# Chemical118/TREW

Measured on NVIDIA B200. Metric: Gbases/s for trew short 5 32 at 1/2/4/8 B200; % of HBM roofline, higher is better.
Workload: dtype u64

## Files before the change

trew_b200/csrc/exact_thread.cuh:

```cuda
#pragma once
#include <stdint.h>

#if defined(__CUDACC__)
#define ET_HD __host__ __device__ __forceinline__
#define ET_FN __host__ __device__ __noinline__
#else
#define ET_HD inline
#define ET_FN inline
#endif

namespace trew {
namespace et {

typedef uint32_t u32;
typedef uint64_t u64;
typedef unsigned __int128 u128;

constexpr int kReadWords = 5;
constexpr int kMaxRead = 32 * kReadWords;
constexpr int kClsCap = 6;
constexpr int kClsSpill = kMaxRead - kClsCap;
constexpr int kApproxMaxWindows = 48;

enum {
    W_H = 0, W_L = W_H + kReadWords + 2, W_V = W_L + kReadWords + 2,
    W_PH = W_V + kReadWords, W_PL = W_PH + kReadWords + 2,
    W_WV = W_PL + kReadWords + 2, W_LINK = W_WV + kReadWords,
    W_CKEY = W_LINK + kReadWords
};
template <class K>
struct Lay {
    static constexpr int KW = (int)(sizeof(K) / 4);
    static constexpr int CT = W_CKEY + KW * kClsCap, WORDS = CT + kClsCap;
};
constexpr int kWorkWords = Lay<u64>::WORDS;

struct Mem {
    u32* base; int stride;
    ET_HD u32& operator[](int i) const { return base[i * stride]; }
};

ET_HD int popc(u32 x) {
#if defined(__CUDA_ARCH__)
    return __popc(x);
#else
    return __builtin_popcount(x);
#endif
}
ET_HD int ffs1(u32 x) {
#if defined(__CUDA_ARCH__)
    return __ffs(x) - 1;
#else
    return __builtin_ctz(x);
#endif
}
ET_HD u32 fshr(u32 lo, u32 hi, int sh) {
#if defined(__CUDA_ARCH__)
    return __funnelshift_r(lo, hi, sh);
#else
    sh &= 31;
    return sh ? (lo >> sh) | (hi << (32 - sh)) : lo;
#endif
}
ET_HD u32 brev32(u32 x) {
#if defined(__CUDA_ARCH__)
    return __brev(x);
#else
    x = ((x >> 1) & 0x55555555u) | ((x & 0x55555555u) << 1);
    x = ((x >> 2) & 0x33333333u) | ((x & 0x33333333u) << 2);
    x = ((x >> 4) & 0x0f0f0f0fu) | ((x & 0x0f0f0f0fu) << 4);
    x = ((x >> 8) & 0x00ff00ffu) | ((x & 0x00ff00ffu) << 8);
    return (x >> 16) | (x << 16);
#endif
}
ET_HD u32 lowmask(int bits) { return bits >= 32 ? 0xffffffffu : (bits <= 0 ? 0u : ((1u << bits) - 1u)); }
ET_HD u32 pxor32(u32 x) { x ^= x << 1; x ^= x << 2; x ^= x << 4; x ^= x << 8; x ^= x << 16; return x; }
ET_HD u64 spread(u32 x) {
    u64 v = x;
    v = (v | (v << 16)) & 0x0000FFFF0000FFFFULL;
    v = (v | (v << 8)) & 0x00FF00FF00FF00FFULL;
    v = (v | (v << 4)) & 0x0F0F0F0F0F0F0F0FULL;
    v = (v | (v << 2)) & 0x3333333333333333ULL;
    v = (v | (v << 1)) & 0x5555555555555555ULL;
    return v;
}

ET_FN u64 canon64(u64 w, int k) {
    const int sh = 2 * (k - 1);
    if (k <= 16) {
        u32 b = (u32)w, c = (u32)w;
        for (int r = 1; r < k; r++) { c = ((c & 3u) << sh) | (c >> 2); b = c < b ? c : b; }
        return b;
    }
    u64 best = w, cur = w;
    for (int r = 1; r < k; r++) { cur = ((cur & 3ULL) << sh) | (cur >> 2); best = cur < best ? cur : best; }
    return best;
}
ET_FN u128 canon128(u128 w, int k) {
    const int sh = 2 * (k - 1);
    u128 best = w, cur = w;
    for (int r = 1; r < k; r++) { cur = ((cur & 3) << sh) | (cur >> 2); best = cur < best ? cur : best; }
    return best;
}
ET_HD u64 canon(u64 w, int k) { return canon64(w, k); }
ET_HD u128 canon(u128 w, int k) { return k <= 32 ? (u128)canon64((u64)w, k) : canon128(w, k); }
ET_HD u64 crc(u64 w, int k) {
    const u32 lo = brev32((u32)w), hi = brev32((u32)(w >> 32));
    u64 x = ((u64)lo << 32) | hi;
    x = ((x >> 1) & 0x5555555555555555ULL) | ((x & 0x5555555555555555ULL) << 1);
    return canon64(~x >> (64 - 2 * k), k);
}
ET_HD u128 crc(u128 w, int k) {
    if (k <= 32) return (u128)crc((u64)w, k);
    u128 r = 0;
    for (int i = 0; i < k; i++) { r = (r << 2) | (3 - (w & 3)); w >>= 2; }
    return canon128(r, k);
}
ET_HD bool homo(u64 w, int k) {
    return k <= 1 || ((w ^ (w >> 2)) & ((1ULL << (2 * (k - 1))) - 1ULL)) == 0;
}
ET_HD bool homo(u128 w, int k) {
    return k <= 1 || ((w ^ (w >> 2)) & ((((u128)1) << (2 * (k - 1))) - 1)) == 0;
}

template <class K>
struct ClsSpill {
    K key[kClsSpill];
    unsigned short tot[kClsSpill], last[kClsSpill];
};

template <class K>
ET_HD K cls_key(Mem m, int q) {
    K v = 0;
    for (int i = Lay<K>::KW - 1; i >= 0; i--) v = (v << 16 << 16) | (K)m[W_CKEY + Lay<K>::KW * q + i];
    return v;
}
template <class K>
ET_HD void cls_put(Mem m, int q, K key) {
    for (int i = 0; i < Lay<K>::KW; i++) { m[W_CKEY + Lay<K>::KW * q + i] = (u32)key; key = key >> 16 >> 16; }
}

ET_HD u32 shr_plane(Mem m, int base, int j, int k) {
    if (k < 32) return fshr(m[base + j], m[base + j + 1], k);
    if (k == 32) return m[base + j + 1];
    if (k < 64) return fshr(m[base + j + 1], m[base + j + 2], k - 32);
    return m[base + j + 2];
}

ET_HD u64 raw_kmer(Mem m, int j, int b, int k, u64& hk, u64& lk, u64) {
    const u32 km = lowmask(k);
    const u32 h = fshr(m[W_H + j], m[W_H + j + 1], b) & km, l = fshr(m[W_L + j], m[W_L + j + 1], b) & km;
    hk = h; lk = l;
    return (spread(brev32(h) >> (32 - k)) << 1) | spread(brev32(l) >> (32 - k));
}
ET_HD u128 raw_kmer(Mem m, int j, int b, int k, u64& hk, u64& lk, u128) {
    if (k <= 32) return (u128)raw_kmer(m, j, b, k, hk, lk, (u64)0);
    const u64 km = k >= 64 ? ~0ULL : ((1ULL << k) - 1ULL);
    hk = ((u64)fshr(m[W_H + j], m[W_H + j + 1], b) | ((u64)fshr(m[W_H + j + 1], m[W_H + j + 2], b) << 32)) & km;
    lk = ((u64)fshr(m[W_L + j], m[W_L + j + 1], b) | ((u64)fshr(m[W_L + j + 1], m[W_L + j + 2], b) << 32)) & km;
    const u64 hr = (((u64)brev32((u32)hk) << 32) | brev32((u32)(hk >> 32))) >> (64 - k);
    const u64 lr = (((u64)brev32((u32)lk) << 32) | brev32((u32)(lk >> 32))) >> (64 - k);
    const u64 lo = (spread((u32)hr) << 1) | spread((u32)lr), hi = (spread((u32)(hr >> 32)) << 1) | spread((u32)(lr >> 32));
    return ((u128)hi << 64) | lo;
}

ET_HD u32 run_starts(Mem m, int j) {
    return m[W_WV + j] & ~((m[W_LINK + j] << 1) | (j ? m[W_LINK + j - 1] >> 31 : 0u));
}
ET_FN int prepare_runs(Mem m, int nw, int k) {
    for (int j = 0; j < nw; j++) {
        const u32 hs = shr_plane(m, W_H, j, k), ls = shr_plane(m, W_L, j, k);
        const u32 eq = ~((hs ^ m[W_H + j]) | (ls ^ m[W_L + j]));
        const u32 wvj = m[W_WV + j];
        const u32 nxt = (wvj >> 1) | (j + 1 < nw ? m[W_WV + j + 1] << 31 : 0u);
        m[W_LINK + j] = eq & wvj & nxt;
    }
    int runs = 0;
    for (int j = 0; j < nw; j++) runs += popc(run_starts(m, j));
    return runs;
}

template <class K>
ET_FN int classify_runs(Mem m, int runs, int k, ClsSpill<K>& x, bool approx, int T = 0, int need_min = 0) {
    int n = 0, ord = 0, j = 0, best = 0;
    const int slack = T - need_min;
    u32 wvj = m[W_WV], rr = run_starts(m, 0);
    for (int r = 0; r < runs; r++) {
        while (!rr) { ord += popc(wvj); j++; rr = run_starts(m, j); wvj = m[W_WV + j]; }
        {
            const int b = ffs1(rr);
            rr &= rr - 1;
            const u32 c0 = (u32)(ord + popc(wvj & ((1u << b) - 1u)));
            int jj = j;
            u32 z = ~m[W_LINK + j] & (0xffffffffu << b);
            while (!z) { jj++; z = ~m[W_LINK + jj]; }
            const u32 cnt = (u32)(32 * (jj - j) + ffs1(z) - b + 1);
            u64 hk, lk;
            K key = raw_kmer(m, j, b, k, hk, lk, (K)0);
            if (approx) key = (K)((u32)(popc((u32)hk) + popc((u32)(hk >> 32))) | ((u32)(popc((u32)lk) + popc((u32)(lk >> 32))) << 8) |
                                  ((u32)(popc((u32)(hk & lk)) + popc((u32)((hk & lk) >> 32))) << 16));
            else key = canon(key, k);
            const u32 last = c0 + cnt - 1u;
            int q = 0;
            const int nq = n < kClsCap ? n : kClsCap;
            while (q < nq && cls_key<K>(m, q) != key) q++;
            u32 tot = cnt;
            if (q < nq) {
                const u32 ct = (m[Lay<K>::CT + q] & 0xffff0000u) + (cnt << 16);
                m[Lay<K>::CT + q] = ct | last;
                tot = ct >> 16;
            } else if (n < kClsCap) {
                cls_put<K>(m, n, key); m[Lay<K>::CT + n] = (cnt << 16) | last;
                n++;
            } else {
                int s = 0;
                while (s < n - kClsCap && x.key[s] != key) s++;
                if (s < n - kClsCap) { tot = x.tot[s] + cnt; x.tot[s] = (unsigned short)tot; x.last[s] = (unsigned short)last; }
                else { x.key[s] = key; x.tot[s] = (unsigned short)cnt; x.last[s] = (unsigned short)last; n++; }
            }
            if (need_min > 0) {
                best = (int)tot > best ? (int)tot : best;
                if ((int)last + 1 - best > slack) return -1;
            }
        }
    }
    return n;
}

template <class K>
ET_FN int cls_max(Mem m, int n, const ClsSpill<K>& x, K& S) {
    u32 best = 0;
    S = 0;
    for (int q = 0; q < n && q < kClsCap; q++) {
        const u32 ct = m[Lay<K>::CT + q];
        const u32 score = ((ct >> 16) << 10) | (1023u - (ct & 0xffffu));
        if (score > best) { best = score; S = cls_key<K>(m, q); }
    }
    for (int q = 0; q < n - kClsCap; q++) {
        const u32 score = ((u32)x.tot[q] << 10) | (1023u - x.last[q]);
        if (score > best) { best = score; S = x.key[q]; }
    }
    return (int)(best >> 10);
}

ET_HD bool need_pass(const unsigned short* thr, u32 need, int M, int T) {
    const u32 mm = need & 0xffffu, t = need >> 16;
    return M >= (int)thr[T] && (t == 0u || (u32)M * t >= mm * (u32)T);
}

ET_HD int min_accept(const unsigned short* thr, u32 need, int T) {
    const u32 mm = need & 0xffffu, t = need >> 16;
    const int a = (int)thr[T], b = t ? (int)((mm * (u32)T + t - 1u) / t) : 0;
    return a > b ? a : b;
}

ET_HD void shrink_valid(Mem m, int nw) {
    for (int j = 0; j < nw; j++) m[W_WV + j] &= (m[W_WV + j] >> 1) | (j + 1 < nw ? m[W_WV + j + 1] << 31 : 0u);
}

template <class K>
ET_FN u32 scan_window(Mem m, int len, int kmin, int kmax, const unsigned short* thr_low, const unsigned short* thr_high, ClsSpill<K>& x,
                      K& S_h, K& S_l) {
    S_h = S_l = 0;
    if (kmax > len) kmax = len;
    if (kmax < kmin) return 0u;
    const int nw = (len + 31) >> 5;
    {
        u32 ch = 0, cl = 0, tph = 0, tpl = 0;
        for (int j = 0; j <= nw; j++) {
            const u32 ih = pxor32(m[W_H + j]) ^ ch, il = pxor32(m[W_L + j]) ^ cl;
            m[W_PH + j] = (ih << 1) | tph; m[W_PL + j] = (il << 1) | tpl;
            tph = ih >> 31; tpl = il >> 31;
            ch = 0u - tph; cl = 0u - tpl;
        }
        m[W_PH + nw + 1] = 0u; m[W_PL + nw + 1] = 0u;
    }
    for (int j = 0; j < nw; j++) m[W_WV + j] = m[W_V + j];
    for (int t = 1; t < kmin; t++) shrink_valid(m, nw);
    K blockedL = 0, blockedH = 0;
    u32 needL = 0, needH = 0;
    u32 res = 0;
    for (int k = kmin; k <= kmax; k++, shrink_valid(m, nw)) {
        const bool blkL = (bool)((blockedL >> k) & 1), blkH = (bool)((blockedH >> k) & 1);
        int T = 0, cH = 0, cL = 0, c11 = 0;
        for (int j = 0; j < nw; j++) {
            const u32 wvj = m[W_WV + j];
            const u32 dh = (shr_plane(m, W_PH, j, k) ^ m[W_PH + j]) & wvj;
            const u32 dl = (shr_plane(m, W_PL, j, k) ^ m[W_PL + j]) & wvj;
            T += popc(wvj); cH += popc(dh); cL += popc(dl); c11 += popc(dh & dl);
        }
        if (T == 0) break;
        if (blkL && blkH) continue;
        const int c10 = cH - c11, c01 = cL - c11, c00 = T - cH - cL + c11;
        int U = c00 > c01 ? c00 : c01;
        U = U > c10 ? U : c10;
        U = U > c11 ? U : c11;
        if (!((!blkL && need_pass(thr_low, needL, U, T)) || (!blkH && need_pass(thr_high, needH, U, T)))) continue;
        K S;
        const int runs = prepare_runs(m, nw, k);
        int need_min = 1 << 20;
        if (!blkL) need_min = min_accept(thr_low, needL, T);
        if (!blkH) { const int a = min_accept(thr_high, needH, T); need_min = a < need_min ? a : need_min; }
        if (runs > 3 && T <= kApproxMaxWindows) {
            const int na = classify_runs(m, runs, k, x, true, T, need_min);
            if (na < 0) continue;
            const int Mu = cls_max(m, na, x, S);
            if (!((!blkL && need_pass(thr_low, needL, Mu, T)) || (!blkH && need_pass(thr_high, needH, Mu, T)))) continue;
        }
        const int n = classify_runs(m, runs, k, x, false, T, need_min);
        if (n < 0) continue;
        const int M = cls_max(m, n, x, S);
        if (homo(S, k)) continue;
        const bool accL = !blkL && need_pass(thr_low, needL, M, T), accH = !blkH && need_pass(thr_high, needH, M, T);
        if (accL || accH) {
            K mm = 0;
            for (int j = k; j <= kmax; j += k) mm |= ((K)1) << j;
            const u32 need = (u32)M | ((u32)T << 16);
            if (accL) { res = (res & 0xffu) | ((u32)k << 8); needL = need; blockedL |= mm; S_l = S; }
            if (accH) { res = (res & 0xff00u) | (u32)k; needH = need; blockedH |= mm; S_h = S; }
        }
    }
    return res;
}

enum { T_F = 0, T_B = 2, T_O = 4 };

template <class K, class Emit>
ET_HD void emit_window_classes(Mem m, int len, int k, int table, bool folded, ClsSpill<K>& x, Emit& emit);

template <class K, class Load, class Emit>
ET_HD bool route_short_thread(Mem m, int n, u32 pm, int min_mer, int max_mer, const unsigned short* thr_low,
                              const unsigned short* thr_high, Load& load, Emit& emit) {
    if (n < 2 * min_mer) return true;
    if (max_mer > (int)(4 * sizeof(K)) || n > kMaxRead) return false;
    const int kmax = n / 4 < max_mer ? n / 4 : max_mer;
    const int llen = n / 2, rlen = (n + 1) / 2, roff = n - rlen;
    ClsSpill<K> x;
    u32 L = 0, R = 0;
    K sh, sl;
    const bool halves = n >= 4 * min_mer;
    for (u32 todo = halves ? pm & 3u : 0u; todo != 0u; todo &= todo - 1u) {
        const bool right = (todo & 1u) == 0u;
        const int len = right ? rlen : llen;
        load(0, right ? roff : 0, len);
        const u32 r = scan_window(m, len, min_mer, kmax, thr_low, thr_high, x, sh, sl);
        if (right) R = r; else L = r;
    }
    if (4 * max_mer > n) {
        const bool hc0 = ((L | R) & 0xffu) == 0u, hc1 = ((L | R) >> 8) == 0u;
        const u32 wbit = halves ? 4u : 1u;
        if ((hc0 || hc1) && (pm & wbit)) {
            const int lo = n / 4 + 1 > min_mer ? n / 4 + 1 : min_mer, hi = n / 2 < max_mer ? n / 2 : max_mer;
            load(0, 0, n);
            const u32 W = scan_window(m, n, lo, hi, thr_low, thr_high, x, sh, sl);
            for (int c = 0; c < 2; c++) {
                const int k = (int)((W >> (8 * c)) & 0xffu);
                if ((c == 0 ? hc0 : hc1) && k) emit_window_classes(m, n, k, T_O + c, false, x, emit);
            }
        }
    }
    if ((L | R) == 0u) return true;
    int cur_win = -1, cur_k = 0, ncls = 0, T = 0;
    for (int c = 0; c < 2; c++) {
        const int Lc = (int)((L >> (8 * c)) & 0xffu), Rc = (int)((R >> (8 * c)) & 0xffu);
        int win, k, table;
        if (Lc > 0 && Lc == Rc) { win = 2; k = Lc; table = T_O + c; }
        else if (Lc > 0) { win = 0; k = Lc; table = T_F + c; }
        else if (Rc > 0) { win = 1; k = Rc; table = T_B + c; }
        else continue;
        if (win != cur_win || k != cur_k) {
            const int off = win == 1 ? roff : 0, len = win == 2 ? n : (win == 0 ? llen : rlen), nw = (len + 31) >> 5;
            load(0, off, len);
            for (int j = 0; j < nw; j++) m[W_WV + j] = m[W_V + j];
            for (int t = 1; t < k; t++) shrink_valid(m, nw);
            T = 0;
            for (int j = 0; j < nw; j++) T += popc(m[W_WV + j]);
            ncls = 0;
            if (T) ncls = classify_runs(m, prepare_runs(m, nw, k), k, x, false);
            cur_win = win; cur_k = k;
        }
        if (T == 0) continue;
        const bool target = win == 2;
        if (target) {
            K S;
            const int M = cls_max(m, ncls, x, S);
            if (homo(S, k) || M < (int)(c == 0 ? thr_high : thr_low)[T]) continue;
        }
        for (int q = 0; q < ncls; q++) {
            K key = q < kClsCap ? cls_key<K>(m, q) : x.key[q - kClsCap];
            const u64 cnt = q < kClsCap ? (u64)(m[Lay<K>::CT + q] >> 16) : (u64)x.tot[q - kClsCap];
            if (target) { const K t = crc(key, k); key = t < key ? t : key; }
            emit(table, k, key, cnt);
        }
    }
    return true;
}

template <class K, class Emit>
ET_HD void emit_window_classes(Mem m, int len, int k, int table, bool folded, ClsSpill<K>& x, Emit& emit) {
    const int nw = (len + 31) >> 5;
    for (int j = 0; j < nw; j++) m[W_WV + j] = m[W_V + j];
    for (int t = 1; t < k; t++) shrink_valid(m, nw);
    int T = 0;
    for (int j = 0; j < nw; j++) T += popc(m[W_WV + j]);
    if (T == 0) return;
    const int ncls = classify_runs(m, prepare_runs(m, nw, k), k, x, false);
    for (int q = 0; q < ncls; q++) {
        K key = q < kClsCap ? cls_key<K>(m, q) : x.key[q - kClsCap];
        const u64 cnt = q < kClsCap ? (u64)(m[Lay<K>::CT + q] >> 16) : (u64)x.tot[q - kClsCap];
        if (folded) { const K t = crc(key, k); key = t < key ? t : key; }
        emit(table, k, key, cnt);
    }
}

template <class K, class Load, class Emit>
ET_HD bool route_pair_thread(Mem m, int n1, int n2, int min_mer, int max_mer, const unsigned short* thr_low,
                             const unsigned short* thr_high, Load& load, Emit& emit) {
    const int n = n1 < n2 ? n1 : n2;
    if (n < 2 * min_mer) return true;
    if (max_mer > (int)(4 * sizeof(K)) || n1 > kMaxRead || n2 > kMaxRead || 4 * max_mer > n) return false;
    const int kmax = n / 4 < max_mer ? n / 4 : max_mer;
    const int soff[5] = {0, 0, n1 - (n1 + 1) / 2, n2 - (n2 + 1) / 2, 0};
    const int slen[5] = {0, n1 / 2, (n1 + 1) / 2, (n2 + 1) / 2, n2 / 2};
    ClsSpill<K> x;
    u32 res[5] = {0, 0, 0, 0, 0};
    K S[5][2];
    bool have[5] = {false, false, false, false, false};
    auto window = [&](int t) { load(t <= 2 ? 0 : 1, soff[t], slen[t]); };
    auto scan = [&](int t) {
        if (have[t]) return;
        window(t);
        res[t] = scan_window(m, slen[t], min_mer, kmax, thr_low, thr_high, x, S[t][0], S[t][1]);
        have[t] = true;
    };
    int pseg[2][8], ptmp[2][8], np[2] = {0, 0};
    int si[2] = {1, 1}, km[2] = {0, 0};
    bool ended[2] = {false, false};
    K ks[2] = {0, 0};
    for (int ti = 1; ti <= 4 && !(ended[0] && ended[1]); ti++) {
        scan(ti);
        for (int c = 0; c < 2; c++) {
            const int k = (int)((res[ti] >> (8 * c)) & 0xffu);
            if (!ended[c] && k) { pseg[c][np[c]] = ti; ptmp[c][np[c]] = ti <= 2 ? 0 : 1; np[c]++; }
            bool ok = !ended[c] && k > 0;
            if (ok && ti != 1) {
                const K ds = ti > 2 ? crc(S[ti][c], k) : S[ti][c];
                ok = km[c] == k && ks[c] == ds;
            }
            if (ok) { si[c]++; km[c] = k; if (ti == 1) ks[c] = S[ti][c]; }
            else ended[c] = true;
        }
    }
    for (int c = 0; c < 2; c++) {
        if (si[c] == 5) {
            for (int e = 0; e < np[c]; e++) {
                const int sg = pseg[c][e];
                window(sg);
                emit_window_classes(m, slen[sg], (int)((res[sg] >> (8 * c)) & 0xffu), T_O + c, true, x, emit);
            }
        }
    }
    if (si[0] <= 4 || si[1] <= 4) {
        int sj[2] = {4, 4};
        km[0] = km[1] = 0; ended[0] = ended[1] = false;
        for (int tj = 4; tj >= 1 && !(ended[0] && ended[1]); tj--) {
            scan(tj);
            for (int c = 0; c < 2; c++) {
                const int k = (int)((res[tj] >> (8 * c)) & 0xffu);
                if (!ended[c] && k) { pseg[c][np[c]] = tj; ptmp[c][np[c]] = tj <= 2 ? 1 : 0; np[c]++; }
                bool ok = sj[c] >= si[c] && !ended[c] && k > 0;
                if (ok && tj != 4) {
                    const K ds = tj <= 2 ? crc(S[tj][c], k) : S[tj][c];
                    ok = km[c] == k && ks[c] == ds;
                }
                if (ok) { sj[c]--; km[c] = k; if (tj == 4) ks[c] = S[tj][c]; }
                else ended[c] = true;
            }
        }
    }
    for (int c = 0; c < 2; c++) {
        if (si[c] <= 4) {
            for (int e = 0; e < np[c]; e++) {
                const int sg = pseg[c][e];
                window(sg);
                emit_window_classes(m, slen[sg], (int)((res[sg] >> (8 * c)) & 0xffu), (ptmp[c][e] == 0 ? T_F : T_B) + c, false, x, emit);
            }
        }
    }
    return true;
}


struct LongGeom {
    int n, SL, snum, mid, bonus;
    ET_HD LongGeom(int n_, int SL_) : n(n_), SL(SL_), snum(n_ / SL_), mid((n_ / SL_ + 1) / 2), bonus(n_ % SL_) {}
    ET_HD int start(int t) const { return (t - 1) * SL + (t > mid ? bonus : 0); }
    ET_HD int len(int t) const { return SL + (t == mid ? bonus : 0); }
};

template <class Load>
ET_HD u32 long_slice_stats(Mem m, const LongGeom& g, int t, int min_mer, int max_mer, const unsigned short* thr_low,
                           const unsigned short* thr_high, Load& load, ClsSpill<u64>& x) {
    const int len = g.len(t);
    load(0, g.start(t), len);
    u64 sh, sl;
    return scan_window(m, len, min_mer, max_mer, thr_low, thr_high, x, sh, sl);
}

struct LongTask { unsigned short slice; unsigned char k, table_folded; };

template <class Stat, class Task>
ET_HD bool long_walk(const LongGeom& g, Stat& stat, Task& task) {
    const int snum = g.snum;
    const bool mid_ok = g.len(g.mid) <= kMaxRead;
    for (int pass = mid_ok ? 1 : 0; pass < 2; pass++) {
        int si[2] = {1, 1}, km[2] = {0, 0};
        bool ended[2] = {false, false};
        int nf = 0;
        for (int ti = 1; ti <= snum && !(ended[0] && ended[1]); ti++) {
            if (pass == 0 && ti == g.mid) return false;
            const u32 r = stat(ti);
            for (int c = 0; c < 2; c++) {
                const int k = (int)((r >> (8 * c)) & 0xffu);
                if (!ended[c] && k > 0 && (ti == 1 || km[c] == k)) { si[c]++; km[c] = k; }
                else ended[c] = true;
            }
            nf = ti;
        }
        if (pass == 1) {
            bool en[2] = {false, false};
            int kk[2] = {0, 0};
            const bool full[2] = {si[0] == snum + 1, si[1] == snum + 1};
            for (int ti = 1; ti <= nf; ti++) {
                const u32 r = stat(ti);
                for (int c = 0; c < 2; c++) {
                    const int k = (int)((r >> (8 * c)) & 0xffu);
                    if (!en[c] && k) task(LongTask{(unsigned short)ti, (unsigned char)k, (unsigned char)(((full[c] ? T_O : T_F) + c) | (full[c] ? 8 : 0))});
                    if (!en[c] && k > 0 && (ti == 1 || kk[c] == k)) kk[c] = k;
                    else en[c] = true;
                }
            }
        }
        if (si[0] <= snum || si[1] <= snum) {
            int sj[2] = {snum, snum};
            km[0] = km[1] = 0; ended[0] = ended[1] = false;
            for (int tj = snum; tj >= 1 && !(ended[0] && ended[1]); tj--) {
                if (pass == 0 && tj == g.mid) return false;
                const u32 r = stat(tj);
                for (int c = 0; c < 2; c++) {
                    const int k = (int)((r >> (8 * c)) & 0xffu);
                    if (pass == 1 && !ended[c] && k) task(LongTask{(unsigned short)tj, (unsigned char)k, (unsigned char)(T_B + c)});
                    if (sj[c] >= si[c] && !ended[c] && k > 0 && (tj == snum || km[c] == k)) { sj[c]--; km[c] = k; }
                    else ended[c] = true;
                }
            }
        }
    }
    return true;
}

template <class Load, class Emit>
ET_HD void long_emit(Mem m, const LongGeom& g, const LongTask& tk, Load& load, ClsSpill<u64>& x, Emit& emit) {
    const int len = g.len(tk.slice);
    load(0, g.start(tk.slice), len);
    emit_window_classes(m, len, tk.k, tk.table_folded & 7, (tk.table_folded & 8) != 0, x, emit);
}

}
}
```

Baseline: 986.2.

## Keep period planes in registers and memoize raw-kmer class lookups

The prefix-xor planes and the valid-window mask move out of strided scratch memory into fixed-size register arrays. A templated scan with compile-time word count (3 words for short windows) and unrolled signature counting replaces the strided loads. classify_runs adds a small memo of raw k-mers that maps repeats straight to their class slot, skipping canonicalisation and the linear key search. The blocked-period masks shrink to a narrower bit set. Together these cut local/global memory traffic and ALU work, at the cost of more register pressure and code size from the template instantiations.

```diff
diff --git a/trew_b200/csrc/exact_thread.cuh b/trew_b200/csrc/exact_thread.cuh
--- a/trew_b200/csrc/exact_thread.cuh
+++ b/trew_b200/csrc/exact_thread.cuh
@@ -8,6 +8,13 @@
 #define ET_HD inline
 #define ET_FN inline
 #endif
+#if defined(__CUDA_ARCH__)
+#define ET_UNROLL _Pragma("unroll")
+#define ET_NO_UNROLL _Pragma("unroll 1")
+#else
+#define ET_UNROLL
+#define ET_NO_UNROLL
+#endif
 
 namespace trew {
 namespace et {
@@ -24,8 +31,7 @@
 
 enum {
     W_H = 0, W_L = W_H + kReadWords + 2, W_V = W_L + kReadWords + 2,
-    W_PH = W_V + kReadWords, W_PL = W_PH + kReadWords + 2,
-    W_WV = W_PL + kReadWords + 2, W_LINK = W_WV + kReadWords,
+    W_WV = W_V + kReadWords, W_LINK = W_WV + kReadWords,
     W_CKEY = W_LINK + kReadWords
 };
 template <class K>
@@ -180,10 +186,20 @@
     return runs;
 }
 
+constexpr int kMemo = 4;
+#if defined(ET_MEMO_STATS) && !defined(__CUDA_ARCH__)
+inline long memo_runs = 0, memo_hits = 0;
+#define ET_MEMO_COUNT(hit) (memo_runs++, memo_hits += (hit) >= 0)
+#else
+#define ET_MEMO_COUNT(hit) ((void)0)
+#endif
 template <class K>
 ET_FN int classify_runs(Mem m, int runs, int k, ClsSpill<K>& x, bool approx, int T = 0, int need_min = 0) {
     int n = 0, ord = 0, j = 0, best = 0;
     const int slack = T - need_min;
+    K mraw[kMemo];
+    u32 mcls = 0;
+    int nm = 0;
     u32 wvj = m[W_WV], rr = run_starts(m, 0);
     for (int r = 0; r < runs; r++) {
         while (!rr) { ord += popc(wvj); j++; rr = run_starts(m, j); wvj = m[W_WV + j]; }
@@ -196,27 +212,50 @@
             while (!z) { jj++; z = ~m[W_LINK + jj]; }
             const u32 cnt = (u32)(32 * (jj - j) + ffs1(z) - b + 1);
             u64 hk, lk;
-            K key = raw_kmer(m, j, b, k, hk, lk, (K)0);
-            if (approx) key = (K)((u32)(popc((u32)hk) + popc((u32)(hk >> 32))) | ((u32)(popc((u32)lk) + popc((u32)(lk >> 32))) << 8) |
-                                  ((u32)(popc((u32)(hk & lk)) + popc((u32)((hk & lk) >> 32))) << 16));
-            else key = canon(key, k);
+            const K raw = raw_kmer(m, j, b, k, hk, lk, (K)0);
             const u32 last = c0 + cnt - 1u;
-            int q = 0;
-            const int nq = n < kClsCap ? n : kClsCap;
-            while (q < nq && cls_key<K>(m, q) != key) q++;
+            int hit = -1;
+            if (!approx) {
+ET_UNROLL
+                for (int e = 0; e < kMemo; e++) hit = e < nm && mraw[e] == raw ? (int)((mcls >> (8 * e)) & 0xffu) : hit;
+            }
+            if (!approx) ET_MEMO_COUNT(hit);
             u32 tot = cnt;
-            if (q < nq) {
-                const u32 ct = (m[Lay<K>::CT + q] & 0xffff0000u) + (cnt << 16);
-                m[Lay<K>::CT + q] = ct | last;
+            if (hit >= kClsCap) {
+                const int s = hit - kClsCap;
+                tot = x.tot[s] + cnt; x.tot[s] = (unsigned short)tot; x.last[s] = (unsigned short)last;
+            } else if (hit >= 0) {
+                const u32 ct = (m[Lay<K>::CT + hit] & 0xffff0000u) + (cnt << 16);
+                m[Lay<K>::CT + hit] = ct | last;
                 tot = ct >> 16;
-            } else if (n < kClsCap) {
-                cls_put<K>(m, n, key); m[Lay<K>::CT + n] = (cnt << 16) | last;
-                n++;
             } else {
-                int s = 0;
-                while (s < n - kClsCap && x.key[s] != key) s++;
-                if (s < n - kClsCap) { tot = x.tot[s] + cnt; x.tot[s] = (unsigned short)tot; x.last[s] = (unsigned short)last; }
-                else { x.key[s] = key; x.tot[s] = (unsigned short)cnt; x.last[s] = (unsigned short)last; n++; }
+                K key;
+                if (approx) key = (K)((u32)(popc((u32)hk) + popc((u32)(hk >> 32))) | ((u32)(popc((u32)lk) + popc((u32)(lk >> 32))) << 8) |
+                                      ((u32)(popc((u32)(hk & lk)) + popc((u32)((hk & lk) >> 32))) << 16));
+                else key = canon(raw, k);
+                int q = 0;
+                const int nq = n < kClsCap ? n : kClsCap;
+                while (q < nq && cls_key<K>(m, q) != key) q++;
+                if (q < nq) {
+                    const u32 ct = (m[Lay<K>::CT + q] & 0xffff0000u) + (cnt << 16);
+                    m[Lay<K>::CT + q] = ct | last;
+                    tot = ct >> 16;
+                } else if (n < kClsCap) {
+                    cls_put<K>(m, n, key); m[Lay<K>::CT + n] = (cnt << 16) | last;
+                    n++;
+                } else {
+                    int s = 0;
+                    while (s < n - kClsCap && x.key[s] != key) s++;
+                    if (s < n - kClsCap) { tot = x.tot[s] + cnt; x.tot[s] = (unsigned short)tot; x.last[s] = (unsigned short)last; }
+                    else { x.key[s] = key; x.tot[s] = (unsigned short)cnt; x.last[s] = (unsigned short)last; n++; }
+                    q = kClsCap + s;
+                }
+                if (!approx && nm < kMemo) {
+ET_UNROLL
+                    for (int e = 0; e < kMemo; e++) if (e == nm) mraw[e] = raw;
+                    mcls |= (u32)q << (8 * nm);
+                    nm++;
+                }
             }
             if (need_min > 0) {
                 best = (int)tot > best ? (int)tot : best;
@@ -258,45 +297,67 @@
     for (int j = 0; j < nw; j++) m[W_WV + j] &= (m[W_WV + j] >> 1) | (j + 1 < nw ? m[W_WV + j + 1] << 31 : 0u);
 }
 
-template <class K>
-ET_FN u32 scan_window(Mem m, int len, int kmin, int kmax, const unsigned short* thr_low, const unsigned short* thr_high, ClsSpill<K>& x,
-                      K& S_h, K& S_l) {
-    S_h = S_l = 0;
-    if (kmax > len) kmax = len;
-    if (kmax < kmin) return 0u;
+template <int NW>
+ET_HD void shrink_valid(u32 (&wv)[NW]) {
+ET_UNROLL
+    for (int j = 0; j < NW; j++) wv[j] &= (wv[j] >> 1) | (j + 1 < NW ? wv[j + 1] << 31 : 0u);
+}
+template <int S, int NW>
+ET_HD void sig_counts(const u32 (&ph)[NW + 2], const u32 (&pl)[NW + 2], const u32 (&wv)[NW], int k, int& cH, int& cL, int& c11) {
+ET_UNROLL
+    for (int j = 0; j < NW; j++) {
+        const u32 dh = (fshr(ph[S + j], S + j + 1 < NW + 2 ? ph[S + j + 1] : 0u, k) ^ ph[j]) & wv[j];
+        const u32 dl = (fshr(pl[S + j], S + j + 1 < NW + 2 ? pl[S + j + 1] : 0u, k) ^ pl[j]) & wv[j];
+        cH += popc(dh); cL += popc(dl); c11 += popc(dh & dl);
+    }
+}
+
+template <class K> struct PeriodSet { typedef u64 T; };
+template <> struct PeriodSet<u64> { typedef u32 T; };
+
+template <class K, int NW>
+ET_HD u32 scan_periods(Mem m, int len, int kmin, int kmax, const unsigned short* thr_low, const unsigned short* thr_high, ClsSpill<K>& x,
+                       K (&S)[2]) {
     const int nw = (len + 31) >> 5;
+    u32 ph[NW + 2], pl[NW + 2], wv[NW];
     {
         u32 ch = 0, cl = 0, tph = 0, tpl = 0;
-        for (int j = 0; j <= nw; j++) {
+ET_UNROLL
+        for (int j = 0; j <= NW; j++) {
             const u32 ih = pxor32(m[W_H + j]) ^ ch, il = pxor32(m[W_L + j]) ^ cl;
-            m[W_PH + j] = (ih << 1) | tph; m[W_PL + j] = (il << 1) | tpl;
+            ph[j] = (ih << 1) | tph; pl[j] = (il << 1) | tpl;
             tph = ih >> 31; tpl = il >> 31;
             ch = 0u - tph; cl = 0u - tpl;
         }
-        m[W_PH + nw + 1] = 0u; m[W_PL + nw + 1] = 0u;
-    }
-    for (int j = 0; j < nw; j++) m[W_WV + j] = m[W_V + j];
-    for (int t = 1; t < kmin; t++) shrink_valid(m, nw);
-    K blockedL = 0, blockedH = 0;
+        ph[NW + 1] = 0u; pl[NW + 1] = 0u;
+    }
+ET_UNROLL
+    for (int j = 0; j < NW; j++) wv[j] = j < nw ? m[W_V + j] : 0u;
+    for (int t = 1; t < kmin; t++) shrink_valid<NW>(wv);
+    typedef typename PeriodSet<K>::T Set;
+    Set blockedL = 0, blockedH = 0;
     u32 needL = 0, needH = 0;
     u32 res = 0;
-    for (int k = kmin; k <= kmax; k++, shrink_valid(m, nw)) {
-        const bool blkL = (bool)((blockedL >> k) & 1), blkH = (bool)((blockedH >> k) & 1);
+ET_NO_UNROLL
+    for (int k = kmin; k <= kmax; k++, shrink_valid<NW>(wv)) {
+        const bool blkL = (bool)((blockedL >> (k - 1)) & 1u), blkH = (bool)((blockedH >> (k - 1)) & 1u);
         int T = 0, cH = 0, cL = 0, c11 = 0;
-        for (int j = 0; j < nw; j++) {
-            const u32 wvj = m[W_WV + j];
-            const u32 dh = (shr_plane(m, W_PH, j, k) ^ m[W_PH + j]) & wvj;
-            const u32 dl = (shr_plane(m, W_PL, j, k) ^ m[W_PL + j]) & wvj;
-            T += popc(wvj); cH += popc(dh); cL += popc(dl); c11 += popc(dh & dl);
-        }
+ET_UNROLL
+        for (int j = 0; j < NW; j++) T += popc(wv[j]);
         if (T == 0) break;
         if (blkL && blkH) continue;
+        if (k < 32) sig_counts<0, NW>(ph, pl, wv, k, cH, cL, c11);
+        else if constexpr (sizeof(K) == 8) sig_counts<1, NW>(ph, pl, wv, k, cH, cL, c11);
+        else if (k < 64) sig_counts<1, NW>(ph, pl, wv, k, cH, cL, c11);
+        else sig_counts<2, NW>(ph, pl, wv, k, cH, cL, c11);
         const int c10 = cH - c11, c01 = cL - c11, c00 = T - cH - cL + c11;
         int U = c00 > c01 ? c00 : c01;
         U = U > c10 ? U : c10;
         U = U > c11 ? U : c11;
         if (!((!blkL && need_pass(thr_low, needL, U, T)) || (!blkH && need_pass(thr_high, needH, U, T)))) continue;
-        K S;
+        K Sk;
+ET_UNROLL
+        for (int j = 0; j < NW; j++) m[W_WV + j] = wv[j];
         const int runs = prepare_runs(m, nw, k);
         int need_min = 1 << 20;
         if (!blkL) need_min = min_accept(thr_low, needL, T);
@@ -304,23 +365,32 @@
         if (runs > 3 && T <= kApproxMaxWindows) {
             const int na = classify_runs(m, runs, k, x, true, T, need_min);
             if (na < 0) continue;
-            const int Mu = cls_max(m, na, x, S);
+            const int Mu = cls_max(m, na, x, Sk);
             if (!((!blkL && need_pass(thr_low, needL, Mu, T)) || (!blkH && need_pass(thr_high, needH, Mu, T)))) continue;
         }
         const int n = classify_runs(m, runs, k, x, false, T, need_min);
         if (n < 0) continue;
-        const int M = cls_max(m, n, x, S);
-        if (homo(S, k)) continue;
+        const int M = cls_max(m, n, x, Sk);
+        if (homo(Sk, k)) continue;
         const bool accL = !blkL && need_pass(thr_low, needL, M, T), accH = !blkH && need_pass(thr_high, needH, M, T);
         if (accL || accH) {
-            K mm = 0;
-            for (int j = k; j <= kmax; j += k) mm |= ((K)1) << j;
+            Set mm = 0;
+            for (int j = k; j <= kmax; j += k) mm |= ((Set)1) << (j - 1);
             const u32 need = (u32)M | ((u32)T << 16);
-            if (accL) { res = (res & 0xffu) | ((u32)k << 8); needL = need; blockedL |= mm; S_l = S; }
-            if (accH) { res = (res & 0xff00u) | (u32)k; needH = need; blockedH |= mm; S_h = S; }
+            if (accL) { res = (res & 0xffu) | ((u32)k << 8); needL = need; blockedL |= mm; S[1] = Sk; }
+            if (accH) { res = (res & 0xff00u) | (u32)k; needH = need; blockedH |= mm; S[0] = Sk; }
         }
     }
     return res;
+}
+template <class K>
+ET_FN u32 scan_window(Mem m, int len, int kmin, int kmax, const unsigned short* thr_low, const unsigned short* thr_high, ClsSpill<K>& x,
+                      K (&S)[2]) {
+    S[0] = S[1] = 0;
+    if (kmax > len) kmax = len;
+    if (kmax < kmin) return 0u;
+    if (len <= 96) return scan_periods<K, 3>(m, len, kmin, kmax, thr_low, thr_high, x, S);
+    return scan_periods<K, kReadWords>(m, len, kmin, kmax, thr_low, thr_high, x, S);
 }
 
 enum { T_F = 0, T_B = 2, T_O = 4 };
@@ -337,13 +407,13 @@
     const int llen = n / 2, rlen = (n + 1) / 2, roff = n - rlen;
     ClsSpill<K> x;
     u32 L = 0, R = 0;
-    K sh, sl;
+    K S[2];
     const bool halves = n >= 4 * min_mer;
     for (u32 todo = halves ? pm & 3u : 0u; todo != 0u; todo &= todo - 1u) {
         const bool right = (todo & 1u) == 0u;
         const int len = right ? rlen : llen;
         load(0, right ? roff : 0, len);
-        const u32 r = scan_window(m, len, min_mer, kmax, thr_low, thr_high, x, sh, sl);
+        const u32 r = scan_window(m, len, min_mer, kmax, thr_low, thr_high, x, S);
         if (right) R = r; else L = r;
     }
     if (4 * max_mer > n) {
@@ -352,7 +422,7 @@
         if ((hc0 || hc1) && (pm & wbit)) {
             const int lo = n / 4 + 1 > min_mer ? n / 4 + 1 : min_mer, hi = n / 2 < max_mer ? n / 2 : max_mer;
             load(0, 0, n);
-            const u32 W = scan_window(m, n, lo, hi, thr_low, thr_high, x, sh, sl);
+            const u32 W = scan_window(m, n, lo, hi, thr_low, thr_high, x, S);
             for (int c = 0; c < 2; c++) {
                 const int k = (int)((W >> (8 * c)) & 0xffu);
                 if ((c == 0 ? hc0 : hc1) && k) emit_window_classes(m, n, k, T_O + c, false, x, emit);
@@ -430,7 +500,7 @@
     auto scan = [&](int t) {
         if (have[t]) return;
         window(t);
-        res[t] = scan_window(m, slen[t], min_mer, kmax, thr_low, thr_high, x, S[t][0], S[t][1]);
+        res[t] = scan_window(m, slen[t], min_mer, kmax, thr_low, thr_high, x, S[t]);
         have[t] = true;
     };
     int pseg[2][8], ptmp[2][8], np[2] = {0, 0};
@@ -503,8 +573,8 @@
                            const unsigned short* thr_high, Load& load, ClsSpill<u64>& x) {
     const int len = g.len(t);
     load(0, g.start(t), len);
-    u64 sh, sl;
-    return scan_window(m, len, min_mer, max_mer, thr_low, thr_high, x, sh, sl);
+    u64 S[2];
+    return scan_window(m, len, min_mer, max_mer, thr_low, thr_high, x, S);
 }
 
 struct LongTask { unsigned short slice; unsigned char k, table_folded; };
```

Measured after the change: 1035 (median of 6 runs). 1.05x the previous value.
